# privacy-scaling-explorations/zkevm-specs

Measured on AMD Instinct MI355X. Metric: BN254 constraint-rows/sec, higher is better.
Workload: dtype u256 (BN254 Fr: 4xu64 canonical cells, u32-limb Montgomery); 1 GPU; EVM circuit, 2^18 execution steps per GPU, mixed-opcode synthetic trace (BASELINE configs[2]); RW table 816377 rows, bytecode table 43913 rows; steps_per_gpu=262144, rw_rows=816377, bytecode_rows=43913, witness_copies=3

## Files before the change

### zkevm_specs_amd/csrc/cpu_backend.cpp

```cpp
#include <stdio.h>
#include <string.h>
#include <chrono>
#include <functional>
#include <string>
#include <vector>

#include "../../include/zkevm_hip.h"
#include "dist_tally.hpp"
#include "state_circuit.hpp"
#include "evm_circuit.hpp"
#include "host_index.hpp"
#include "row_circuits.hpp"
#include "copy_circuit.hpp"
#include "sign_circuit.hpp"
#include "keccak_table.hpp"
#include "secp256k1.hpp"
#include "pi_circuit.hpp"
#include "state_assign.hpp"
#include "bytecode_assign.hpp"
#include "bytecode_code.hpp"
#include "block_tables.hpp"
#include "trace_witness.hpp"
#include "state_rekey.hpp"
#include "ecc_circuit.hpp"
// ... 384 lines not shown
    cpu_table(s->tab[1], t->bytecode, nullptr, t->n_bytecode, BYTECODE_NCELLS, bc_key_hash);
    cpu_table(s->tab[2], t->tx, t->tx_flags, t->n_tx, TX_NCELLS, tx_key_hash);
    cpu_table(s->tab[3], t->block, t->block_flags, t->n_block, BLOCK_NCELLS, blk_key_hash);
    cpu_table(s->tab[4], t->copy, nullptr, t->n_copy, COPY_T_NCELLS, copy_key_hash);
    cpu_table(s->tab[5], t->keccak, nullptr, t->n_keccak, KECCAK_NCELLS, keccak_key_hash);
    cpu_table(s->tab[6], t->exp, nullptr, t->n_exp, EXP_T_NCELLS, expt_key_hash);
    cpu_table(s->tab[7], t->sig, nullptr, t->n_sig, SIG_T_NCELLS, sig_key_hash);
    cpu_table(s->tab[8], t->ecc, nullptr, t->n_ecc, ECC_T_NCELLS, ecc_key_hash);
    cpu_table(s->tab[9], t->withdrawals, nullptr, t->n_withdrawals, 4, nullptr);
    a.rw = s->tab[0].t; a.bytecode = s->tab[1].t; a.tx = s->tab[2].t; a.block = s->tab[3].t; a.copy = s->tab[4].t;
    a.keccak = s->tab[5].t; a.exp = s->tab[6].t; a.sig = s->tab[7].t; a.ecc = s->tab[8].t; a.withdrawals = s->tab[9].t;
    {
        const HostEvmAgg g = evm_aggregates_host(t->tx, t->tx_flags, t->n_tx, t->withdrawals, t->n_withdrawals);
        a.agg_max_txs = g.max_txs; a.agg_total_txs = g.total_txs; a.agg_invalid_txs = g.invalid_txs;
        a.agg_bad_invalid_rows = g.bad_invalid_rows; a.agg_total_wds = g.total_wds;
        a.agg_rw_dups = rw_duplicate_rows_host(t->rw, t->n_rw);
    }
    a.aux = nullptr;
    a.aux_kind = nullptr;
    a.aux_cells = t->aux_cells ? t->aux_cells : 2u;
    if (t->aux && t->aux_kind) {
        s->aux64.assign(t->aux, t->aux + t->n_steps * a.aux_cells * 4);
        s->a32[1].assign(t->aux_kind, t->aux_kind + t->n_steps);
        a.aux = s->aux64.data();
        a.aux_kind = s->a32[1].data();
    }
    a.perm = nullptr;
    a.prof = nullptr;
    a.n_pairs = (u32)(t->n_steps - 1);
    a.opts = (t->begin_with_first_step ? 1u : 0u) | (t->end_with_last_step ? 2u : 0u);
    a.rw_dense = 0;
    a.rw_base = 0;
    a.rw_keys = nullptr;
    a.codes.n = 0;
    a.codes.mask = 0;
    a.codes.packed = nullptr;
    a.codes.entries = nullptr;
    a.codes.slots = nullptr;
    if (!(opts & ZK_OPT_GENERIC_INDEX)) {
        s->rw_meta = rw_dense_meta_host(s->tab[0].t.n ? s->tab[0].cells.data() : nullptr, t->n_rw);
        a.rw_dense = s->rw_meta.dense;
        a.rw_base = s->rw_meta.base;
        if (s->rw_meta.dense) {
            s->a64[1].resize((size_t)t->n_rw * 4);
            for (u64 r = 0; r < t->n_rw; r++) {
                const RwKey k = rw_pack_row(a.rw, (u32)r);
                for (int j = 0; j < 4; j++) s->a64[1][4 * r + j] = k.w[j];
            }
            a.rw_keys = s->a64[1].data();
        }
        if (t->n_bytecode) {
            build_code_dir(s->tab[1].cells.data(), t->n_bytecode, s->dir);
            a.codes.entries = s->dir.entries.data();
            a.codes.slots = s->dir.slots.data();
            a.codes.mask = s->dir.mask;
            a.codes.n = (u32)s->dir.entries.size();
            a.codes.packed = s->dir.packed.data();
        }
    }
    s->row = [s](u64 i) {
        u32 c = evm_check_step<EVM_GROUP_ALL>(s->evm, i);
        if (c == ZK_NOT_MINE) c = evm_check_step<EVM_GROUP_WARM>(s->evm, i);
        if (c == ZK_NOT_MINE) c = evm_check_step<EVM_GROUP_COLD>(s->evm, i);
        return c;
    };
    *out = s;
    return 0;
}
extern "C" int zk_evm_verify(const zk_evm_tables* t, uint32_t opts, uint32_t* status_out, zk_result* result) {
    ARG_TRY(result, "zk_evm_verify: result is null");
    zk_session* s = nullptr;
    const int rc = zk_evm_open(t, opts, &s);
    return rc ? rc : one_shot(s, status_out, result);
}

extern "C" int zk_evm_verify_batch(const zk_evm_tables* const* t, uint64_t n, uint32_t opts, zk_result* results) {
    ARG_TRY((t && results) || n == 0, "zk_evm_verify_batch: bad arguments");
    for (uint64_t i = 0; i < n; i++) ARG_TRY(t[i], "zk_evm_verify_batch: null witness");
    for (uint64_t i = 0; i < n; i++) {
        const int rc = zk_evm_verify(t[i], opts, nullptr, &results[i]);
        if (rc) return rc;
    }
// ... 1946 lines not shown
```

### zkevm_specs_amd/csrc/evm_circuit.hpp

```cpp
#pragma once
#include "common.hpp"
#include "evm_tables.h"
#include "keccak.hpp"
#include "secp_constants.h"
#include "bigz.hpp"

enum { S_STATE = 0, S_RWC, S_CALL_ID, S_IS_ROOT, S_IS_CREATE, S_CH_LO, S_CH_HI, S_PC, S_SP, S_GAS, S_MWS, S_REV, S_LOG, STEP_NCELLS };
enum { R_RWC = 0, R_RW, R_TAG, R_ID, R_ADDR, R_FT, R_KEY_LO, R_KEY_HI, R_VAL_LO, R_VAL_HI, R_PREV_LO, R_PREV_HI, R_AUX_LO, R_AUX_HI, RW_NCELLS };
enum { B_HASH_LO = 0, B_HASH_HI, B_TAG, B_INDEX, B_IS_CODE, B_VALUE, BYTECODE_NCELLS };
enum { TX_NCELLS = 5, BLOCK_NCELLS = 4 };
enum { CT_IS_FIRST = 0, CT_SRC_ID_LO, CT_SRC_ID_HI, CT_SRC_TAG, CT_DST_ID_LO, CT_DST_ID_HI, CT_DST_TAG, CT_SRC_ADDR,
       CT_SRC_ADDR_END, CT_DST_ADDR, CT_LENGTH, CT_RLC_ACC, CT_RWC, CT_RWC_INC, COPY_T_NCELLS };
enum { XT_IS_STEP = 0, XT_ID, XT_IS_LAST, XT_BASE0, XT_BASE1, XT_BASE2, XT_BASE3, XT_EXP_LO, XT_EXP_HI, XT_RES_LO, XT_RES_HI,
       EXP_T_NCELLS };
enum { SIG_T_NCELLS = 9, ECC_T_NCELLS = 13 };
enum { AUX_PAIR = 3, AUX_ECRECOVER = 5, AUX_ECADD = 6, AUX_ECMUL = 7, AUX_ECPAIRING = 8 };
enum { CDT_Bytecode = 1, CDT_Memory, CDT_TxCalldata, CDT_TxLog, CDT_RlcAcc };

struct EvmDyn {
    u32 rw_sparse;
    u32 codes_n;
    u64 rw_base;
    u32 codes_mask;
    u32 agg_max_txs, agg_total_txs, agg_invalid_txs, agg_bad_invalid_rows, agg_total_wds;
    u32 dir_entries;
    u32 n_deferred;
    u32 agg_rw_dups;
};

struct EvmArgs {
    const EvmDyn* dyn;
    const u64* steps;
    const u32* step_recs;
    u64 n_steps;
    ZkTable rw, bytecode, tx, block;
    ZkTable copy, keccak, exp;
    ZkTable sig, ecc;
    ZkTable withdrawals;
    u32 agg_max_txs, agg_total_txs, agg_invalid_txs, agg_bad_invalid_rows, agg_total_wds;
    u32 agg_rw_dups;
    const u64* aux;
    const u32* aux_kind;
    u32 aux_cells;
    u32 rw_dense;
    u64 rw_base;
    const u64* rw_keys;
    ZkCodeDir codes;
    unsigned long long* prof;
    u32* defer_list;
    u32* defer_count;
    const u32* perm;
    u32 n_pairs;
    u32 opts;
    u32* defer_count_twin;
};

ZK_HD void evm_args_resolve(EvmArgs& a) {
#ifdef EVM_RESOLVE_OFF
    return;
#endif
    if (a.dyn) {
        const EvmDyn d = *a.dyn;
        a.rw_dense = (a.rw.n != 0u && d.rw_sparse == 0u) ? 1u : 0u;
        a.rw_base = d.rw_base;
        a.codes.n = d.codes_n;
        a.codes.mask = d.codes_mask;
        a.agg_max_txs = d.agg_max_txs; a.agg_total_txs = d.agg_total_txs; a.agg_invalid_txs = d.agg_invalid_txs;
        a.agg_bad_invalid_rows = d.agg_bad_invalid_rows; a.agg_total_wds = d.agg_total_wds;
        a.agg_rw_dups = d.agg_rw_dups;
    }
}

#ifndef EVM_HOT_BLOCK
#define EVM_HOT_BLOCK 128
#endif
#define EVM_STAGE_LANES EVM_HOT_BLOCK
#define EV_PROF_WAVE ((blockIdx.x * blockDim.x + threadIdx.x) >> 6)
#define EV_PROF_ON(a) ((a).prof && (threadIdx.x & 63) == 0 && EV_PROF_WAVE < 4096u)
#define EVM_STAGE_STRIDE (EVM_STAGE_LANES + 1)
#define EVM_STAGE_ENTRIES 40
#define EVM_STAGE_GAS 10
ZK_HD constexpr int evm_stage_entry(int s, int c) {
    return c == S_CH_LO || c == S_CH_HI ? 24 + s * 8 + (c - S_CH_LO) * 4
           : s * 12 + (c < S_CH_LO ? c : c == S_PC ? 5 : c == S_SP ? 6 : c == S_MWS ? 7 : c == S_REV ? 8 : c == S_LOG ? 9 : EVM_STAGE_GAS);
}
#define EVM_DIR_MAX_SLOTS 128
#define EVM_DIR_MAX_ENTRIES 32
// ... 291 lines not shown
    Q.q[c] = v;
    Q.mask |= 1u << c;
}
ZK_HD void rwq_set_word(RwQ& Q, int c, const Word& w) {
    rwq_set(Q, c, w.lo);
    rwq_set(Q, c + 1, w.hi);
}
struct RwKey {
    u64 w[4];
};
ZK_HD bool rw_key_fields_fit(const Fr& rw, const Fr& tag, const Fr& id, const Fr& addr, const Fr& ft) {
    return fr_le_u64(rw, 255) && fr_le_u64(tag, 255) && fr_le_u64(ft, 255) && fr_fits64(id) && (addr.v[5] | addr.v[6] | addr.v[7]) == 0u;
}
ZK_HD RwKey rw_pack_fields(const Fr& rw, const Fr& tag, const Fr& id, const Fr& addr, const Fr& ft) {
    RwKey k;
    k.w[0] = (1ull << 63) | (u64)(rw.v[0] & 0xffu) | ((u64)(tag.v[0] & 0xffu) << 8) | ((u64)(ft.v[0] & 0xffu) << 16) | ((u64)addr.v[4] << 24);
    k.w[1] = fr_lo64(id);
    k.w[2] = fr_lo64(addr);
    k.w[3] = fr_hi64of128(addr);
    return k;
}
ZK_HD RwKey rw_pack_row(const ZkTable& t, u32 r) {
    const Fr rw = zk_table_cell(t, r, R_RW), tag = zk_table_cell(t, r, R_TAG), id = zk_table_cell(t, r, R_ID);
    const Fr addr = zk_table_cell(t, r, R_ADDR), ft = zk_table_cell(t, r, R_FT);
    if (!rw_key_fields_fit(rw, tag, id, addr, ft)) {
        RwKey k;
        k.w[0] = k.w[1] = k.w[2] = k.w[3] = 0;
        return k;
    }
    RwKey k = rw_pack_fields(rw, tag, id, addr, ft);
    k.w[0] |= (u64)((t.flags ? t.flags[r] : 3u) & 3u) << 56;
    return k;
}
ZK_HD u32 rw_dense_row(const EvmArgs& a, const Fr& rwc, bool& ok) {
    const u64 off = fr_lo64(rwc) - a.rw_base;
    ok = fr_fits64(rwc) && fr_lo64(rwc) >= a.rw_base && off < (u64)a.rw.n;
    return ok ? (u32)off : 0u;
}
struct RwRow {
    uint4 k01, k23;
    Fr v_lo, v_hi;
    u32 r;
};
template <int N>
struct RwRows {
    bool valid;
    RwRow row[N];
};
ZK_HD u32 rw_lookup(Ins& I, RwQ& Q, const Fr* rw_counter = nullptr, const RwRow* pre = nullptr) {
    if (rw_counter) {
        Q.q[R_RWC] = *rw_counter;
    } else {
        Q.q[R_RWC] = fr_add_u64(I.rwc, I.rw_off);
        I.rw_off++;
    }
    if (I.a->rw_dense) {
        I.seq++;
        bool ok;
        const u32 r = rw_dense_row(*I.a, Q.q[R_RWC], ok);
        bool key_cells = true;
#if EVM_FAST
        if (!I.a->rw_keys) I.defer = 3u;
#endif
        if (I.a->rw_keys) {
            uint4 k01, k23;
            if (pre) {
                if (pre->r != r && I.err == 0u) I.err = ZK_CODE(ZK_UNSUPPORTED, I.seq);
                k01 = pre->k01;
                k23 = pre->k23;
            } else {
                const uint4* kp = reinterpret_cast<const uint4*>(I.a->rw_keys + (u64)r * 4);
                k01 = kp[0];
                k23 = kp[1];
            }
            const u64 w0 = (u64)k01.x | ((u64)k01.y << 32), w1 = (u64)k01.z | ((u64)k01.w << 32);
            const u64 w2 = (u64)k23.x | ((u64)k23.y << 32), w3 = (u64)k23.z | ((u64)k23.w << 32);
            if (w0 >> 63) {
                const u32 m = Q.mask;
                if ((m >> R_RW) & 1u) ok = ok & (fr_le_u64(Q.q[R_RW], 255) & ((u32)(w0 & 0xffu) == Q.q[R_RW].v[0]));
                if ((m >> R_TAG) & 1u) ok = ok & (fr_le_u64(Q.q[R_TAG], 255) & ((u32)((w0 >> 8) & 0xffu) == Q.q[R_TAG].v[0]));
                if ((m >> R_FT) & 1u) ok = ok & (fr_le_u64(Q.q[R_FT], 255) & ((u32)((w0 >> 16) & 0xffu) == Q.q[R_FT].v[0]));
                if ((m >> R_ID) & 1u) ok = ok & (fr_fits64(Q.q[R_ID]) & (w1 == fr_lo64(Q.q[R_ID])));
                if ((m >> R_ADDR) & 1u) {
                    const Fr& qa = Q.q[R_ADDR];
                    ok = ok & (((qa.v[5] | qa.v[6] | qa.v[7]) == 0u) & (w2 == fr_lo64(qa)) & (w3 == fr_hi64of128(qa)) &
                               ((u32)((w0 >> 24) & 0xffffffffull) == qa.v[4]));
                }
                key_cells = false;
            }
        }
#if EVM_FAST
        if (key_cells) I.defer = 4u;
#else
        if (key_cells) {
#pragma unroll
            for (int c = 1; c <= R_FT; c++)
                if ((Q.mask >> c) & 1u) ok = ok & fr_eq(zk_table_cell(I.a->rw, r, c), Q.q[c]);
        }
#endif
#pragma unroll
        for (int c = R_FT + 1; c < RW_NCELLS; c++)
            if ((Q.mask >> c) & 1u) ok = ok & fr_eq(zk_table_cell(I.a->rw, r, c), Q.q[c]);
        if (!ok) ev_fail(I, ZK_LOOKUP_UNSAT);
        return r;
    }
    return table_lookup<RW_NCELLS>(I, I.a->rw, rw_key_hash_cell(Q.q[R_RWC]), Q.q, Q.mask);
}
template <int N>
ZK_HD void rw_rows_fetch_at(const Ins& I, RwRows<N>& R, u64 off) {
    const EvmArgs& a = *I.a;
    R.valid = a.rw_dense && a.rw_keys != nullptr;
    if (!R.valid) return;
#pragma unroll
    for (int k = 0; k < N; k++) {
        bool ok;
        const u32 r = rw_dense_row(a, fr_add_u64(I.rwc, off + (u64)k), ok);
        const uint4* kp = reinterpret_cast<const uint4*>(a.rw_keys + (u64)r * 4);
        R.row[k].k01 = kp[0];
        R.row[k].k23 = kp[1];
        R.row[k].r = r;
        R.row[k].v_lo = zk_table_cell(a.rw, r, R_VAL_LO);
        R.row[k].v_hi = zk_table_cell(a.rw, r, R_VAL_LO + 1);
    }
}
template <int N>
ZK_HD void rw_rows_fetch(const Ins& I, RwRows<N>& R) { rw_rows_fetch_at(I, R, I.rw_off); }
ZK_HD Fr rw_cell(const Ins& I, u32 row, int c) { return zk_table_cell(I.a->rw, row, c); }
ZK_HD Word rw_word(const Ins& I, u32 row, int c) { return word_of(rw_cell(I, row, c), rw_cell(I, row, c + 1)); }
ZK_HD WordOrValue rw_value(const Ins& I, u32 row) {
    WordOrValue v;
    v.w = rw_word(I, row, R_VAL_LO);
    v.is_word = I.a->rw.flags ? (I.a->rw.flags[row] & 1u) : true;
    return v;
}
ZK_HD WordOrValue rw_value_prev(const Ins& I, u32 row) {
    WordOrValue v;
    v.w = rw_word(I, row, R_PREV_LO);
    v.is_word = I.a->rw.flags ? (I.a->rw.flags[row] & 2u) : true;
    return v;
}

ZK_HD void code_dir_resolve(Ins& I, const Word& code_hash) {
    if (I.code_state != 0) return;
    const ZkCodeDir& dir = I.a->codes;
    I.code_state = 3;
#if !defined(ZK_HOSTSIM)
    static_assert(sizeof(ZkCodeEntry) == 96, "LDS mirror layout: 12 u64 per directory entry");
    if (dir.n != 0 && I.dir_lds && fr_fits128(code_hash.lo) && fr_fits128(code_hash.hi)) {
        u32 slot = (u32)zk_code_hash_key(code_hash.lo, code_hash.hi) & dir.mask;
        I.code_state = 2;
        const u64 h0 = fr_lo64(code_hash.lo), h1 = fr_hi64of128(code_hash.lo), h4 = fr_lo64(code_hash.hi), h5 = fr_hi64of128(code_hash.hi);
        for (u32 probes = 0; probes <= dir.mask; probes++) {
// ... 274 lines not shown
    RwQ Q;
    rwq_init(Q, rw, TG_Stack);
    rwq_set(Q, R_ID, I.call_id);
    const Fr& sp = I.sp;
    rwq_set(Q, R_ADDR, off >= 0 ? fr_add_u64(sp, (u64)off) : fr_sub_u64(sp, (u64)(-off)));
    rw_lookup(I, Q, nullptr, &row);
    return word_of(row.v_lo, row.v_hi);
}
template <int N>
ZK_HD Word stack_pop(Ins& I, const RwRows<N>& R, int k) {
    if (!R.valid) return stack_pop(I);
    int off = I.sp_off;
    I.sp_off++;
    return stack_lookup_row(I, 0, off, R.row[k]);
}
template <int N>
ZK_HD Word stack_push(Ins& I, const RwRows<N>& R, int k) {
    if (!R.valid) return stack_push(I);
    I.sp_off--;
    return stack_lookup_row(I, 1, I.sp_off, R.row[k]);
}
ZK_HD Fr memory_lookup(Ins& I, u32 rw, const Fr& addr, const Fr* call_id = nullptr) {
    RwQ Q;
    rwq_init(Q, rw, TG_Memory);
    rwq_set(Q, R_ID, call_id ? *call_id : I.call_id);
    rwq_set(Q, R_ADDR, addr);
    u32 r = rw_lookup(I, Q);
    return value_of(I, rw_value(I, r));
}
ZK_HD void memory_lookup_run32(Ins& I, u32 rw, const Fr& address) {
    const EvmArgs& a = *I.a;
    const Fr rwc0 = fr_add_u64(I.rwc, I.rw_off);
    const u64 off = fr_lo64(rwc0) - a.rw_base;
    bool fastpath = a.rw_dense && a.rw_keys && fr_fits64(rwc0) && fr_lo64(rwc0) >= a.rw_base && off + 32 <= (u64)a.rw.n && off + 32 > off &&
                    fr_fits64(I.call_id) && (address.v[5] | address.v[6] | address.v[7]) == 0u &&
                    !(address.v[4] == 0xffffffffu && address.v[3] == 0xffffffffu && address.v[2] == 0xffffffffu && address.v[1] == 0xffffffffu &&
                      address.v[0] >= 0xffffffe0u);
    u32 bad_lookup = 0, bad_type = 0;
    if (fastpath) {
        const uint4* kp = reinterpret_cast<const uint4*>(a.rw_keys + off * 4);
        const u64 id = fr_lo64(I.call_id);
#pragma unroll
        for (int b = 0; b < 4; b++) {
            uint4 k01[8], k23[8];
#pragma unroll
            for (int j = 0; j < 8; j++) { k01[j] = kp[2 * (8 * b + j)]; k23[j] = kp[2 * (8 * b + j) + 1]; }
#pragma unroll
            for (int j = 0; j < 8; j++) {
                const int k = 8 * b + j;
                const Fr ak = fr_add_u64(address, (u64)k);
                const u64 w0 = (u64)k01[j].x | ((u64)k01[j].y << 32), w1 = (u64)k01[j].z | ((u64)k01[j].w << 32);
                const u64 w2 = (u64)k23[j].x | ((u64)k23[j].y << 32), w3 = (u64)k23[j].z | ((u64)k23[j].w << 32);
                const u64 want0 = (1ull << 63) | (u64)rw | ((u64)TG_Memory << 8) | ((u64)ak.v[4] << 24);
                const u64 cmp_mask = ~((0xffull << 16) | (3ull << 56));
                if (!(w0 >> 63)) fastpath = false;
                const bool ok = ((w0 ^ want0) & cmp_mask) == 0 && w1 == id && w2 == fr_lo64(ak) && w3 == fr_hi64of128(ak);
                bad_lookup |= (ok ? 0u : 1u) << k;
                bad_type |= (u32)((w0 >> 56) & 1u) << k;
            }
        }
    }
    if (fastpath) {
        for (int k = 0; k < 32; k++) {
            I.seq++;
            if ((bad_lookup >> k) & 1u) ev_fail(I, ZK_LOOKUP_UNSAT);
            I.seq++;
            if ((bad_type >> k) & 1u) ev_fail(I, ZK_ASSERT);
        }
        I.rw_off += 32;
        return;
    }
    for (int k = 0; k < 32; k++) memory_lookup(I, rw, fr_add_u64(address, (u64)k));
}
ZK_HD WordOrValue call_context_lookup_word(Ins& I, u32 field_tag, u32 rw = 0, const Fr* call_id = nullptr) {
    RwQ Q;
    rwq_init(Q, rw, TG_CallContext);
    rwq_set(Q, R_ID, call_id ? *call_id : I.call_id);
    rwq_set(Q, R_ADDR, fr_u(field_tag));
    u32 r = rw_lookup(I, Q);
    return rw_value(I, r);
}
ZK_HD WordOrValue call_context_lookup_word_row(Ins& I, u32 field_tag, u32 rw, const Fr* call_id, const RwRow& row) {
    RwQ Q;
    rwq_init(Q, rw, TG_CallContext);
    rwq_set(Q, R_ID, call_id ? *call_id : I.call_id);
    rwq_set(Q, R_ADDR, fr_u(field_tag));
    const u32 r = rw_lookup(I, Q, nullptr, &row);
    WordOrValue v;
    v.w = word_of(row.v_lo, row.v_hi);
    const u64 w0 = (u64)row.k01.x | ((u64)row.k01.y << 32);
    v.is_word = (w0 >> 63) ? (((w0 >> 56) & 1ull) != 0ull) : (I.a->rw.flags ? (I.a->rw.flags[r] & 1u) : true);
    return v;
}
ZK_HD Fr call_context_lookup(Ins& I, u32 field_tag, u32 rw = 0, const Fr* call_id = nullptr) {
// ... 3580 lines not shown
```

### zkevm_specs_amd/csrc/zkevm_hip.hip

```cpp
#include <hip/hip_runtime.h>
#include <hip/hip_ext.h>
#include <stddef.h>
#include <stdio.h>
#include <string.h>
#include <stdlib.h>
#include <chrono>
#include <memory>
#include <string>
#include <vector>

#include <atomic>
#include <mutex>
#include <dlfcn.h>

#include "../../include/zkevm_hip.h"
#include "kernels.hpp"
#include "dist_tally.hpp"
#include "host_index.hpp"
#include "code_dir_build.hpp"

#define ZK_MAX_DEVICES 64
static std::mutex g_dev_mutex;
static hipStream_t g_own_stream[ZK_MAX_DEVICES] = {nullptr};
static hipStream_t g_batch_stream[ZK_MAX_DEVICES][2] = {{nullptr}};
// ... 220 lines not shown
        if (vblock == 0) {
            if ((k & 127u) == 0) group_start[k >> 7] = gsh[k >> 7] = excl;
            if (k == EVM_N_BINS - 1) group_start[EVM_N_GROUPS] = gsh[EVM_N_GROUPS] = src[k];
            for (u32 j = c_real; j < c; j++) perm[excl + j] = EVM_NO_PAIR;
        }
    }
    const u32 i = vblock * blockDim.x + threadIdx.x;
    u32 bin = 0, rank = 0;
    if (i < n_pairs) {
        bin = bin16[i];
        rank = atomicAdd(&local[bin], 1u);
    }
    __syncthreads();
    if (vblock == 0 && k == 0 && early_host) {
        __hip_atomic_store(&early_host[EVM_EARLY_WORD], gsh[EVM_GROUP_WARM + 1] - gsh[EVM_GROUP_WARM], __ATOMIC_RELAXED, __HIP_MEMORY_SCOPE_SYSTEM);
        __hip_atomic_store(&early_host[EVM_EARLY_WORD + 1], gsh[EVM_GROUP_COLD + 1] - gsh[EVM_GROUP_COLD], __ATOMIC_RELAXED, __HIP_MEMORY_SCOPE_SYSTEM);
        __threadfence_system();
        __hip_atomic_store(&early_host[EVM_EARLY_WORD + 2], early_seq, __ATOMIC_RELEASE, __HIP_MEMORY_SCOPE_SYSTEM);
    }
    if (k < EVM_N_BINS && local[k]) base[k] = excl + atomicAdd(&taken[k], local[k]);
    __syncthreads();
    if (i < n_pairs) perm[base[bin] + rank] = i;
}
__global__ __launch_bounds__(1024) void evm_state_scatter_kernel(const uint16_t* bin16, u32 n_pairs, const u32* hist, u32* hist_next,
                                                                 u32* taken, u32* group_start, u32* perm) {
    evm_state_scatter_body(blockIdx.x, bin16, n_pairs, hist, hist_next, taken, group_start, perm);
}
__global__ __launch_bounds__(256) void evm_open_fill_kernel(uint4* ff, u64 n_ff, uint4* zero, u64 n_zero) {
    const u64 stride = (u64)gridDim.x * blockDim.x;
    const uint4 F = make_uint4(~0u, ~0u, ~0u, ~0u), Z = make_uint4(0u, 0u, 0u, 0u);
    for (u64 i = (u64)blockIdx.x * blockDim.x + threadIdx.x; i < n_ff; i += stride) ff[i] = F;
    for (u64 i = (u64)blockIdx.x * blockDim.x + threadIdx.x; i < n_zero; i += stride) zero[i] = Z;
}
__device__ __forceinline__ void rw_prepare_quad(const ZkTable& t, u64* keys, EvmDyn* dyn, u32 vthread, u32 sparse_bit = 1u) {
    const u32 r = vthread >> 2, q = vthread & 3u;
    const bool in = r < t.n;
    uint4 c0 = make_uint4(0, 0, 0, 0), c1 = c0, c2 = c0;
    u64 base = 0;
    u32 flags = 3u;
    if (in) {
        const uint4* p = reinterpret_cast<const uint4*>(t.cells + (u64)r * RW_NCELLS * 4) + q;
        c0 = p[0];
        c1 = p[4];
        c2 = p[8];
        if (q == 0) {
            base = t.cells[0];
            if (t.flags) flags = t.flags[r];
        }
    }
    bool fit, dense_ok;
    u64 w0 = 0, w1 = 0, w2 = 0, w3 = 0;
    const bool z0hi = (c0.y | c0.z | c0.w) == 0u, z1hi = (c1.y | c1.z | c1.w) == 0u, z2hi = (c2.y | c2.z | c2.w) == 0u;
    const bool z0 = z0hi && c0.x == 0u, z1 = z1hi && c1.x == 0u, z2 = z2hi && c2.x == 0u;
    if (q == 0) {
        const u64 rwc = (u64)c0.x | ((u64)c0.y << 32);
        dense_ok = (c0.z | c0.w) == 0u && rwc == base + r && base + r >= base;
        fit = z1hi && c1.x <= 255u;
        w0 = (u64)(c1.x & 0xffu) << 8 | ((u64)(flags & 3u) << 56) | (1ull << 63);
        w2 = (u64)c2.x | ((u64)c2.y << 32);
        w3 = (u64)c2.z | ((u64)c2.w << 32);
    } else if (q == 1) {
        dense_ok = z0;
        fit = z1 && z2hi;
        w0 = (u64)c2.x << 24;
    } else if (q == 2) {
        dense_ok = true;
        fit = z0hi && c0.x <= 255u && (c1.z | c1.w) == 0u && z2hi && c2.x <= 255u;
        w0 = (u64)(c0.x & 0xffu) | ((u64)(c2.x & 0xffu) << 16);
        w1 = (u64)c1.x | ((u64)c1.y << 32);
    } else {
        dense_ok = true;
        fit = z0 && z1 && z2;
    }
    const u32 qshift = threadIdx.x & 60u;
    const bool fits = ((__ballot(fit) >> qshift) & 0xfull) == 0xfull;
    const unsigned long long nd = __ballot(in && !dense_ok);
    if (nd != 0ull && (threadIdx.x & 63u) == 0) atomicOr(&dyn->rw_sparse, sparse_bit);
    if (r == 0 && q == 0 && in) dyn->rw_base = base;
#pragma unroll
    for (int m = 1; m <= 2; m <<= 1) {
        w0 |= __shfl_xor(w0, m);
        w1 |= __shfl_xor(w1, m);
        w2 |= __shfl_xor(w2, m);
        w3 |= __shfl_xor(w3, m);
    }
    if (!fits) w0 = w1 = w2 = w3 = 0;
    if (in && q < 2) {
        const u64 a = q == 0 ? w0 : w2, b2 = q == 0 ? w1 : w3;
        reinterpret_cast<uint4*>(keys + (u64)r * 4)[q] = make_uint4((u32)a, (u32)(a >> 32), (u32)b2, (u32)(b2 >> 32));
    }
}
#define EVM_OPEN_TABLES 8
struct EvmOpenTables {
    ZkTable t[EVM_OPEN_TABLES];
    u32 block_start[EVM_OPEN_TABLES + 2];
    const u64* wds;
    u32 n_wds;
    EvmDyn* dyn;
    ZkTally* tally;
    ZkTable rw;
    u64* rw_keys;
    u32 dir_block0, rw_block0;
    DirBuild dir;
    const u64* steps;
    u32 n_steps;
    u32* step_recs;
    u32 rec_block0;
    EvmSortArgs sort;
    u32 hist_block0;
    u32 lat_period;
    u32 tail_row0, tail_blocks;
#ifdef ZK_DIAG_P1
    u32 diag_skip;
#endif
};
__device__ __forceinline__ void evm_open_small_tables(const EvmOpenTables& o, u32 block) {
    int k = 0;
#pragma unroll
    for (int j = 1; j <= EVM_OPEN_TABLES; j++) k += block >= o.block_start[j] ? 1 : 0;
    const u32 r = (block - o.block_start[k]) * blockDim.x + threadIdx.x;
    if (k == EVM_OPEN_TABLES) {
        const bool nz = r < o.n_wds && !fr_is_zero(fr_load(o.wds + ((u64)r * 4 + 3) * 4));
        const unsigned long long b = __ballot(nz);
        if (b && (threadIdx.x & 63u) == 0) atomicAdd(&o.dyn->agg_total_wds, (u32)__popcll(b));
        return;
    }
    const ZkTable& t = o.t[k];
    const bool in = r < t.n;
    if (k == 0) {
        bool caller = false, present = false, invalid = false, bad = false;
        if (in) {
            const Fr tag = zk_table_cell(t, r, 1), lo = zk_table_cell(t, r, 3), hi = zk_table_cell(t, r, 4);
            caller = fr_eq_u64(tag, 4);
            present = caller && !(fr_is_zero(lo) && fr_is_zero(hi));
// ... 14 lines not shown
    switch (k) {
    case 0: h = tx_key_hash(t, r); break;
    case 1: h = blk_key_hash(t, r); break;
    case 2: h = bc_key_hash(t, r); break;
    case 3: h = copy_key_hash(t, r); break;
    case 4: h = keccak_key_hash(t, r); break;
    case 5: h = expt_key_hash(t, r); break;
    case 6: h = sig_key_hash(t, r); break;
    default: h = ecc_key_hash(t, r); break;
    }
    u32* slots = const_cast<u32*>(t.slots);
    u32 s = (u32)h & t.mask;
    while (atomicCAS(&slots[s], ZK_EMPTY_SLOT, r) != ZK_EMPTY_SLOT) s = (s + 1) & t.mask;
}
__global__ __launch_bounds__(256) void evm_open_phase1_kernel(EvmOpenTables o) {
    if (blockIdx.x == 0 && threadIdx.x < 2) {
        o.tally[threadIdx.x].fail_count = 0ull;
        o.tally[threadIdx.x].first_fail = ~0ull;
    }
    u32 b = blockIdx.x;
    if (o.lat_period > 1u && b < o.rec_block0) {
        const u32 q = b / o.lat_period;
        b = (b == q * o.lat_period && q < o.rw_block0) ? q : o.rw_block0 + b - (q + 1u < o.rw_block0 ? q + 1u : o.rw_block0);
    }
#ifdef ZK_DIAG_P1
    {
        const u32 range = b < o.dir_block0 ? 1u : b < o.hist_block0 ? 2u : b < o.rw_block0 ? 4u : b < o.rec_block0 ? 8u : 16u;
        if (o.diag_skip & range) return;
    }
#endif
    if (b < o.dir_block0) evm_open_small_tables(o, b);
    else if (b < o.hist_block0) dirb_events_row(o.dir, (b - o.dir_block0) * blockDim.x + threadIdx.x);
    else if (b < o.rw_block0) evm_state_hist_body(b - o.hist_block0, o.sort.steps, o.sort.n_pairs, o.sort.hist, o.sort.taken, o.sort.bin16, o.sort.tally, o.sort.defer_count);
    else if (b < o.rec_block0) rw_prepare_quad(o.rw, o.rw_keys, o.dyn, (b - o.rw_block0) * blockDim.x + threadIdx.x);
    else evm_step_record_quad(o.steps, o.n_steps, o.step_recs, (b - o.rec_block0) * blockDim.x + threadIdx.x);
}
#define EVM_OPEN_RW_GENERIC_BLOCKS 64u
#define EVM_OPEN_P2_BLOCK 1024u
__global__ __launch_bounds__(1024) void evm_open_phase2_kernel(EvmOpenTables o, u32 scatter_blocks, u32 dir_blocks, u32 force_generic) {
    if (blockIdx.x < scatter_blocks) {
        evm_state_scatter_body(blockIdx.x, o.sort.bin16, o.sort.n_pairs, o.sort.hist, o.sort.hist_next, o.sort.taken, o.sort.group_start, o.sort.perm,
                               o.sort.early_host, o.sort.early_seq);
        return;
    }
    const u32 b = blockIdx.x - scatter_blocks;
    if (b < dir_blocks) {
        dirb_finalize_entry(o.dir, b * blockDim.x + threadIdx.x);
        return;
    }
    const u32 generic_blocks = gridDim.x - scatter_blocks - dir_blocks - o.tail_blocks;
    if (b >= dir_blocks + generic_blocks) {
        rw_prepare_quad(o.rw, o.rw_keys, o.dyn, o.tail_row0 * 4u + (b - dir_blocks - generic_blocks) * blockDim.x + threadIdx.x, 2u);
        return;
    }
    if (!force_generic && (o.dyn->rw_sparse & 1u) == 0u) return;
    if (force_generic && b == dir_blocks && threadIdx.x == 0) o.dyn->rw_sparse = 1u;
    u32* slots = const_cast<u32*>(o.rw.slots);
    const u32 stride = generic_blocks * blockDim.x;
    for (u32 r = (b - dir_blocks) * blockDim.x + threadIdx.x; r < o.rw.n; r += stride) {
        u32 s = (u32)rw_key_hash(o.rw, r) & o.rw.mask;
        bool dup = false;
        for (;;) {
            const u32 q = atomicCAS(&slots[s], ZK_EMPTY_SLOT, r);
            if (q == ZK_EMPTY_SLOT) break;
            if (!dup && q < o.rw.n) {
                bool same = true;
                for (int c = 0; c < RW_NCELLS && same; c++) same = fr_eq(zk_table_cell(o.rw, q, c), zk_table_cell(o.rw, r, c));
                dup = same;
            }
            s = (s + 1) & o.rw.mask;
        }
        if (dup) atomicAdd(&o.dyn->agg_rw_dups, 1u);
    }
}

__global__ void fr_op_kernel(int op, const u64* a, const u64* b, u64* out, u64 n) {
    u64 i = (u64)blockIdx.x * blockDim.x + threadIdx.x;
    if (i >= n) return;
    Fr x = fr_load(a + 4 * i), y = fr_load(b + 4 * i), r;
    switch (op) {
    case 0: r = fr_add(x, y); break;
    case 1: r = fr_sub(x, y); break;
    case 2: r = fr_mul(x, y); break;
    case 3: r = fr_mont(x, y); break;
    case 4: r = fr_neg(x); break;
// ... 531 lines not shown
        const size_t zero_bytes = dyn_bytes + 2 * hist_bytes + status_bytes + 3 * (size_t)cap_big * 4;
        char* zero = nullptr;
        if ((rc = dev_alloc(s, (void**)&zero, zero_bytes))) goto fail;
        EvmResultBlock* const rb = (EvmResultBlock*)zero;
        EvmDyn* dyn = &rb->dyn;
        s->d_result = rb;
        if ((rc = arena_pinned(s->device, &s->h_result))) goto fail;
        {
            void* hd = nullptr;
            if (hipHostGetDevicePointer(&hd, s->h_result, 0) == hipSuccess) s->h_result_dev = (u32*)hd;
            (void)hipGetLastError();
        }
        static_assert(sizeof(EvmResultBlock) <= 256, "the result block outgrew its slot");
        static_assert((EVM_N_BINS * sizeof(u32)) % 16 == 0, "zero region pieces are 16-byte multiples");
        s->d_hist = (u32*)(zero + dyn_bytes);
        s->d_hist2 = (u32*)(zero + dyn_bytes + hist_bytes);
        s->d_status = no_status ? nullptr : (u32*)(zero + dyn_bytes + 2 * hist_bytes);
        u32* const dir_last = (u32*)(zero + dyn_bytes + 2 * hist_bytes + status_bytes);
        E.dyn = dyn;
        E.defer_count = &dyn->n_deferred;
        if ((rc = dev_alloc(s, (void**)&E.defer_list, (size_t)E.n_pairs * sizeof(u32)))) goto fail;
        s->d_tally = rb->tally;
        s->tally_last = s->d_tally;
        {
            const u64 n16 = n_ff / 4 + zero_bytes / 16;
            const u32 fill_grid = (u32)(n16 / 256 < 2048 ? (n16 + 255) / 256 : 2048);
            if (arena_event(s->device, &s->ev_open0) || arena_event(s->device, &s->ev_open1)) s->ev_open0 = s->ev_open1 = nullptr;
            hipExtLaunchKernelGGL(evm_open_fill_kernel, dim3(fill_grid ? fill_grid : 1u), dim3(256), 0, s->stream, s->ev_open0, nullptr, 0, (uint4*)ff,
                                  (u64)(n_ff / 4), (uint4*)zero, (u64)(zero_bytes / 16));
        }
        E.rw_dense = 0;
        E.rw_base = 0;
        E.rw_keys = nullptr;
        E.codes.n = 0;
        E.codes.mask = 0;
        E.codes.packed = nullptr;
        E.codes.entries = nullptr;
        E.codes.slots = nullptr;
        E.agg_max_txs = E.agg_total_txs = E.agg_invalid_txs = E.agg_bad_invalid_rows = E.agg_total_wds = E.agg_rw_dups = 0;
        EvmOpenTables o;
        memset(&o, 0, sizeof o);
        u32 blk = 0;
        for (int k = 0; k < EVM_OPEN_TABLES; k++) { o.t[k] = *small[k]; o.block_start[k] = blk; blk += (small[k]->n + 255u) / 256u; }
        o.block_start[EVM_OPEN_TABLES] = blk;
        blk += (u32)((t->n_withdrawals + 255) / 256);
        o.block_start[EVM_OPEN_TABLES + 1] = blk;
        o.wds = E.withdrawals.cells;
        o.n_wds = (u32)t->n_withdrawals;
        o.dyn = dyn;
        o.tally = s->d_tally;
        o.rw = E.rw;
        if (t->n_rw && !generic) {
            u64* d_keys = nullptr;
            if ((rc = dev_alloc(s, (void**)&d_keys, (size_t)t->n_rw * 32))) goto fail;
            E.rw_keys = d_keys;
            o.rw_keys = d_keys;
        }
        u64 n_head = t->n_rw;
        if ((internal & EVM_OPEN_ONESHOT) && o.rw_keys && t->n_rw < (1ull << 30)) {
            static const u32 tail_pm = [] { const char* e = getenv("ZK_P2_RW_TAIL"); const int v = e ? atoi(e) : ZK_P2_RW_TAIL_DEFAULT; return (u32)(v < 0 ? 0 : v > 999 ? 999 : v); }();
            const u64 h = (t->n_rw - t->n_rw * tail_pm / 1000 + 63) & ~63ull;
            if (h < t->n_rw) n_head = h;
        }
        const u32 rw_row_blocks = o.rw_keys ? (u32)((n_head + 63) / 64) : 0u;
        if (n_head < t->n_rw) {
            o.tail_row0 = (u32)n_head;
            o.tail_blocks = (u32)((t->n_rw - n_head + EVM_OPEN_P2_BLOCK / 4 - 1) / (EVM_OPEN_P2_BLOCK / 4));
        }
        o.dir_block0 = blk;
        u32 dir_row_blocks = 0;
        if (want_dir) {
            DirBuild& d = o.dir;
            d.rows = E.bytecode.cells;
            d.n = (u32)t->n_bytecode;
            d.rep = dir_rep;
            d.first = dir_first;
            d.last = dir_last;
            d.runs = dir_last + cap_big;
            d.bad = dir_last + 2 * (size_t)cap_big;
            d.big_mask = cap_big - 1;
            d.small_slots = small_slots;
            d.dyn = dyn;
            if ((rc = dev_alloc(s, (void**)&d.packed, (size_t)d.n * sizeof(uint16_t)))) goto fail;
            if ((rc = dev_alloc(s, (void**)&d.entries, (size_t)DIRB_MAX_ENTRIES * sizeof(ZkCodeEntry)))) goto fail;
            if ((rc = dev_alloc(s, (void**)&d.list, (size_t)DIRB_MAX_ENTRIES * 4))) goto fail;
            dir_row_blocks = (d.n + 255u) / 256u;
            E.codes.entries = d.entries;
            E.codes.slots = d.small_slots;
// ... 3436 lines not shown
```

Measured before the change: 1.656 billion rows/s.

## Split RW lookup keys into a 16-byte primary and an optional high half

```diff
diff --git a/zkevm_specs_amd/csrc/cpu_backend.cpp b/zkevm_specs_amd/csrc/cpu_backend.cpp
--- a/zkevm_specs_amd/csrc/cpu_backend.cpp
+++ b/zkevm_specs_amd/csrc/cpu_backend.cpp
@@ -440,6 +440,7 @@
     a.rw_dense = 0;
     a.rw_base = 0;
     a.rw_keys = nullptr;
+    a.rw_keys16 = a.rw_keys_hi = nullptr;
     a.codes.n = 0;
     a.codes.mask = 0;
     a.codes.packed = nullptr;
@@ -451,11 +452,24 @@
         a.rw_base = s->rw_meta.base;
         if (s->rw_meta.dense) {
             s->a64[1].resize((size_t)t->n_rw * 4);
+#if ZK_RW_KEY16
+            u64* const lo = s->a64[1].data();
+            u64* const hi = lo + (size_t)t->n_rw * 2;
+            for (u64 r = 0; r < t->n_rw; r++) {
+                const RwKey16 k = rw_pack_row16(a.rw, (u32)r);
+                lo[2 * r] = k.a0;
+                lo[2 * r + 1] = k.a1;
+                if (rw_key16_wide(k.a0)) { hi[2 * r] = k.h0; hi[2 * r + 1] = k.h1; }
+            }
+            a.rw_keys16 = lo;
+            a.rw_keys_hi = hi;
+#else
             for (u64 r = 0; r < t->n_rw; r++) {
                 const RwKey k = rw_pack_row(a.rw, (u32)r);
                 for (int j = 0; j < 4; j++) s->a64[1][4 * r + j] = k.w[j];
             }
             a.rw_keys = s->a64[1].data();
+#endif
         }
         if (t->n_bytecode) {
             build_code_dir(s->tab[1].cells.data(), t->n_bytecode, s->dir);
diff --git a/zkevm_specs_amd/csrc/evm_circuit.hpp b/zkevm_specs_amd/csrc/evm_circuit.hpp
--- a/zkevm_specs_amd/csrc/evm_circuit.hpp
+++ b/zkevm_specs_amd/csrc/evm_circuit.hpp
@@ -53,6 +53,8 @@
     u32 n_pairs;
     u32 opts;
     u32* defer_count_twin;
+    const u64* rw_keys16;
+    const u64* rw_keys_hi;
 };
 
 ZK_HD void evm_args_resolve(EvmArgs& a) {
@@ -410,13 +412,88 @@
     k.w[0] |= (u64)((t.flags ? t.flags[r] : 3u) & 3u) << 56;
     return k;
 }
+#ifndef ZK_RW_KEY16
+#define ZK_RW_KEY16 1
+#endif
+#if !ZK_RW_KEY16 || defined(ZK_HOSTSIM)
+#define RW_KEY32_COMPILED 1
+#else
+#define RW_KEY32_COMPILED 0
+#endif
+#ifndef RW_KEY16_HI_SELECT
+#if EVM_FAST
+#define RW_KEY16_HI_SELECT 0
+#else
+#define RW_KEY16_HI_SELECT 1
+#endif
+#endif
+struct RwKey16 {
+    u64 a0, a1, h0, h1;
+};
+ZK_HD bool rw_key16_fits(u64 a0) { return (a0 >> 63) != 0ull; }
+ZK_HD bool rw_key16_wide(u64 a0) { return (a0 >> 62) == 2ull; }
+ZK_HD RwKey16 rw_key16_finish(bool fits, u64 a0, u64 a1, u64 h0, u64 h1) {
+    RwKey16 k;
+    if (!fits) {
+        k.a0 = k.a1 = k.h0 = k.h1 = 0;
+        return k;
+    }
+    k.a0 = a0 | (1ull << 63) | ((h0 | h1) == 0ull ? 1ull << 62 : 0ull);
+    k.a1 = a1;
+    k.h0 = h0;
+    k.h1 = h1;
+    return k;
+}
+ZK_HD RwKey16 rw_pack_row16(const ZkTable& t, u32 r) {
+    const Fr rw = zk_table_cell(t, r, R_RW), tag = zk_table_cell(t, r, R_TAG), id = zk_table_cell(t, r, R_ID);
+    const Fr addr = zk_table_cell(t, r, R_ADDR), ft = zk_table_cell(t, r, R_FT);
+    const u64 a0 = (u64)(rw.v[0] & 0xffu) | ((u64)(tag.v[0] & 0xffu) << 8) | ((u64)(ft.v[0] & 0xffu) << 16) | ((u64)id.v[0] << 24) |
+                   ((u64)((t.flags ? t.flags[r] : 3u) & 3u) << 56);
+    return rw_key16_finish(rw_key_fields_fit(rw, tag, id, addr, ft), a0, fr_lo64(addr), (u64)id.v[1] | ((u64)addr.v[4] << 32), fr_hi64of128(addr));
+}
+ZK_HD bool rw_query_wants_high(const Fr* q, u32 mask) {
+    const bool id_narrow = ((mask >> R_ID) & 1u) && fr_fits64(q[R_ID]) && q[R_ID].v[1] == 0u;
+    const Fr& qa = q[R_ADDR];
+    const bool addr_narrow = ((mask >> R_ADDR) & 1u) && fr_fits64(qa);
+    return !(id_narrow && addr_narrow);
+}
+ZK_HD bool rw_key16_match(u64 a0, u64 a1, u64 h0, u64 h1, const Fr* q, u32 m) {
+    const bool wide = rw_key16_wide(a0);
+    if (!wide) h0 = h1 = 0ull;
+    bool ok = !(wide && !rw_query_wants_high(q, m));
+    if ((m >> R_RW) & 1u) ok = ok & (fr_le_u64(q[R_RW], 255) & ((u32)(a0 & 0xffu) == q[R_RW].v[0]));
+    if ((m >> R_TAG) & 1u) ok = ok & (fr_le_u64(q[R_TAG], 255) & ((u32)((a0 >> 8) & 0xffu) == q[R_TAG].v[0]));
+    if ((m >> R_FT) & 1u) ok = ok & (fr_le_u64(q[R_FT], 255) & ((u32)((a0 >> 16) & 0xffu) == q[R_FT].v[0]));
+    if ((m >> R_ID) & 1u) ok = ok & (fr_fits64(q[R_ID]) & ((u32)(a0 >> 24) == q[R_ID].v[0]) & ((u32)h0 == q[R_ID].v[1]));
+    if ((m >> R_ADDR) & 1u) {
+        const Fr& qa = q[R_ADDR];
+        ok = ok & (((qa.v[5] | qa.v[6] | qa.v[7]) == 0u) & (a1 == fr_lo64(qa)) & (h1 == fr_hi64of128(qa)) & ((u32)(h0 >> 32) == qa.v[4]));
+    }
+    return ok;
+}
+ZK_HD bool rw_keys16_on(const EvmArgs& a) {
+#if ZK_RW_KEY16
+    return a.rw_keys16 != nullptr;
+#else
+    return false;
+#endif
+}
+ZK_HD bool rw_keys_any(const EvmArgs& a) {
+#if RW_KEY32_COMPILED
+    if (a.rw_keys) return true;
+#endif
+    return rw_keys16_on(a);
+}
 ZK_HD u32 rw_dense_row(const EvmArgs& a, const Fr& rwc, bool& ok) {
     const u64 off = fr_lo64(rwc) - a.rw_base;
     ok = fr_fits64(rwc) && fr_lo64(rwc) >= a.rw_base && off < (u64)a.rw.n;
     return ok ? (u32)off : 0u;
 }
 struct RwRow {
-    uint4 k01, k23;
+    uint4 k01;
+#if RW_KEY32_COMPILED
+    uint4 k23;
+#endif
     Fr v_lo, v_hi;
     u32 r;
 };
@@ -438,9 +515,33 @@
         const u32 r = rw_dense_row(*I.a, Q.q[R_RWC], ok);
         bool key_cells = true;
 #if EVM_FAST
-        if (!I.a->rw_keys) I.defer = 3u;
-#endif
-        if (I.a->rw_keys) {
+        if (!rw_keys_any(*I.a)) I.defer = 3u;
+#endif
+#if ZK_RW_KEY16
+        if (I.a->rw_keys16) {
+            const bool want_hi = rw_query_wants_high(Q.q, Q.mask);
+            uint4 k, h;
+            h.x = h.y = h.z = h.w = 0u;
+            if (pre) {
+                if (pre->r != r && I.err == 0u) I.err = ZK_CODE(ZK_UNSUPPORTED, I.seq);
+                k = pre->k01;
+            } else {
+                k = reinterpret_cast<const uint4*>(I.a->rw_keys16)[r];
+            }
+#if RW_KEY16_HI_SELECT
+            h = reinterpret_cast<const uint4*>(want_hi ? I.a->rw_keys_hi : I.a->rw_keys16)[r];
+#else
+            if (want_hi) h = reinterpret_cast<const uint4*>(I.a->rw_keys_hi)[r];
+#endif
+            const u64 a0 = (u64)k.x | ((u64)k.y << 32), a1 = (u64)k.z | ((u64)k.w << 32);
+            if (rw_key16_fits(a0)) {
+                ok = ok & rw_key16_match(a0, a1, (u64)h.x | ((u64)h.y << 32), (u64)h.z | ((u64)h.w << 32), Q.q, Q.mask);
+                key_cells = false;
+            }
+        }
+#endif
+#if RW_KEY32_COMPILED
+        if (!rw_keys16_on(*I.a) && I.a->rw_keys) {
             uint4 k01, k23;
             if (pre) {
                 if (pre->r != r && I.err == 0u) I.err = ZK_CODE(ZK_UNSUPPORTED, I.seq);
@@ -467,6 +568,7 @@
                 key_cells = false;
             }
         }
+#endif
 #if EVM_FAST
         if (key_cells) I.defer = 4u;
 #else
@@ -487,15 +589,25 @@
 template <int N>
 ZK_HD void rw_rows_fetch_at(const Ins& I, RwRows<N>& R, u64 off) {
     const EvmArgs& a = *I.a;
-    R.valid = a.rw_dense && a.rw_keys != nullptr;
+    R.valid = a.rw_dense && rw_keys_any(a);
     if (!R.valid) return;
+    const bool k16 = rw_keys16_on(a);
 #pragma unroll
     for (int k = 0; k < N; k++) {
         bool ok;
         const u32 r = rw_dense_row(a, fr_add_u64(I.rwc, off + (u64)k), ok);
-        const uint4* kp = reinterpret_cast<const uint4*>(a.rw_keys + (u64)r * 4);
-        R.row[k].k01 = kp[0];
-        R.row[k].k23 = kp[1];
+#if RW_KEY32_COMPILED
+        if (!k16) {
+            const uint4* kp = reinterpret_cast<const uint4*>(a.rw_keys + (u64)r * 4);
+            R.row[k].k01 = kp[0];
+            R.row[k].k23 = kp[1];
+        } else {
+            R.row[k].k23.x = R.row[k].k23.y = R.row[k].k23.z = R.row[k].k23.w = 0u;
+        }
+#endif
+#if ZK_RW_KEY16
+        if (k16) R.row[k].k01 = reinterpret_cast<const uint4*>(a.rw_keys16)[r];
+#endif
         R.row[k].r = r;
         R.row[k].v_lo = zk_table_cell(a.rw, r, R_VAL_LO);
         R.row[k].v_hi = zk_table_cell(a.rw, r, R_VAL_LO + 1);
@@ -836,12 +948,39 @@
     const EvmArgs& a = *I.a;
     const Fr rwc0 = fr_add_u64(I.rwc, I.rw_off);
     const u64 off = fr_lo64(rwc0) - a.rw_base;
-    bool fastpath = a.rw_dense && a.rw_keys && fr_fits64(rwc0) && fr_lo64(rwc0) >= a.rw_base && off + 32 <= (u64)a.rw.n && off + 32 > off &&
+    bool fastpath = a.rw_dense && rw_keys_any(a) && fr_fits64(rwc0) && fr_lo64(rwc0) >= a.rw_base && off + 32 <= (u64)a.rw.n && off + 32 > off &&
                     fr_fits64(I.call_id) && (address.v[5] | address.v[6] | address.v[7]) == 0u &&
                     !(address.v[4] == 0xffffffffu && address.v[3] == 0xffffffffu && address.v[2] == 0xffffffffu && address.v[1] == 0xffffffffu &&
                       address.v[0] >= 0xffffffe0u);
     u32 bad_lookup = 0, bad_type = 0;
-    if (fastpath) {
+#if ZK_RW_KEY16
+    if (rw_keys16_on(a)) {
+        fastpath = fastpath && I.call_id.v[1] == 0u && fr_fits64(address) && fr_lo64(address) <= ~31ull;
+        if (fastpath) {
+            const uint4* kp = reinterpret_cast<const uint4*>(a.rw_keys16) + off;
+            const u64 want0 = (3ull << 62) | (u64)rw | ((u64)TG_Memory << 8) | ((u64)I.call_id.v[0] << 24);
+            const u64 cmp_mask = ~((0xffull << 16) | (3ull << 56));
+            const u64 addr0 = fr_lo64(address);
+#pragma unroll
+            for (int b = 0; b < 4; b++) {
+                uint4 kk[8];
+#pragma unroll
+                for (int j = 0; j < 8; j++) kk[j] = kp[8 * b + j];
+#pragma unroll
+                for (int j = 0; j < 8; j++) {
+                    const int k = 8 * b + j;
+                    const u64 a0 = (u64)kk[j].x | ((u64)kk[j].y << 32), a1 = (u64)kk[j].z | ((u64)kk[j].w << 32);
+                    if ((a0 >> 62) != 3ull) fastpath = false;
+                    const bool ok = ((a0 ^ want0) & cmp_mask) == 0 && a1 == addr0 + (u64)k;
+                    bad_lookup |= (ok ? 0u : 1u) << k;
+                    bad_type |= (u32)((a0 >> 56) & 1u) << k;
+                }
+            }
+        }
+    }
+#endif
+#if RW_KEY32_COMPILED
+    if (fastpath && !rw_keys16_on(a)) {
         const uint4* kp = reinterpret_cast<const uint4*>(a.rw_keys + off * 4);
         const u64 id = fr_lo64(I.call_id);
 #pragma unroll
@@ -864,6 +1003,7 @@
             }
         }
     }
+#endif
     if (fastpath) {
         for (int k = 0; k < 32; k++) {
             I.seq++;
diff --git a/zkevm_specs_amd/csrc/zkevm_hip.hip b/zkevm_specs_amd/csrc/zkevm_hip.hip
--- a/zkevm_specs_amd/csrc/zkevm_hip.hip
+++ b/zkevm_specs_amd/csrc/zkevm_hip.hip
@@ -276,7 +276,7 @@
     for (u64 i = (u64)blockIdx.x * blockDim.x + threadIdx.x; i < n_ff; i += stride) ff[i] = F;
     for (u64 i = (u64)blockIdx.x * blockDim.x + threadIdx.x; i < n_zero; i += stride) zero[i] = Z;
 }
-__device__ __forceinline__ void rw_prepare_quad(const ZkTable& t, u64* keys, EvmDyn* dyn, u32 vthread, u32 sparse_bit = 1u) {
+__device__ __forceinline__ void rw_prepare_quad(const ZkTable& t, u64* keys, u64* keys_hi, EvmDyn* dyn, u32 vthread, u32 sparse_bit = 1u) {
     const u32 r = vthread >> 2, q = vthread & 3u;
     const bool in = r < t.n;
     uint4 c0 = make_uint4(0, 0, 0, 0), c1 = c0, c2 = c0;
@@ -300,18 +300,33 @@
         const u64 rwc = (u64)c0.x | ((u64)c0.y << 32);
         dense_ok = (c0.z | c0.w) == 0u && rwc == base + r && base + r >= base;
         fit = z1hi && c1.x <= 255u;
+#if ZK_RW_KEY16
+        w0 = (u64)(c1.x & 0xffu) << 8 | ((u64)(flags & 3u) << 56);
+        w1 = (u64)c2.x | ((u64)c2.y << 32);
+        w3 = (u64)c2.z | ((u64)c2.w << 32);
+#else
         w0 = (u64)(c1.x & 0xffu) << 8 | ((u64)(flags & 3u) << 56) | (1ull << 63);
         w2 = (u64)c2.x | ((u64)c2.y << 32);
         w3 = (u64)c2.z | ((u64)c2.w << 32);
+#endif
     } else if (q == 1) {
         dense_ok = z0;
         fit = z1 && z2hi;
+#if ZK_RW_KEY16
+        w2 = (u64)c2.x << 32;
+#else
         w0 = (u64)c2.x << 24;
+#endif
     } else if (q == 2) {
         dense_ok = true;
         fit = z0hi && c0.x <= 255u && (c1.z | c1.w) == 0u && z2hi && c2.x <= 255u;
         w0 = (u64)(c0.x & 0xffu) | ((u64)(c2.x & 0xffu) << 16);
+#if ZK_RW_KEY16
+        w0 |= (u64)c1.x << 24;
+        w2 = (u64)c1.y;
+#else
         w1 = (u64)c1.x | ((u64)c1.y << 32);
+#endif
     } else {
         dense_ok = true;
         fit = z0 && z1 && z2;
@@ -328,11 +343,17 @@
         w2 |= __shfl_xor(w2, m);
         w3 |= __shfl_xor(w3, m);
     }
+#if ZK_RW_KEY16
+    const RwKey16 k = rw_key16_finish(fits, w0, w1, w2, w3);
+    if (in && q == 0) reinterpret_cast<uint4*>(keys)[r] = make_uint4((u32)k.a0, (u32)(k.a0 >> 32), (u32)k.a1, (u32)(k.a1 >> 32));
+    if (in && q == 1 && rw_key16_wide(k.a0)) reinterpret_cast<uint4*>(keys_hi)[r] = make_uint4((u32)k.h0, (u32)(k.h0 >> 32), (u32)k.h1, (u32)(k.h1 >> 32));
+#else
     if (!fits) w0 = w1 = w2 = w3 = 0;
     if (in && q < 2) {
         const u64 a = q == 0 ? w0 : w2, b2 = q == 0 ? w1 : w3;
         reinterpret_cast<uint4*>(keys + (u64)r * 4)[q] = make_uint4((u32)a, (u32)(a >> 32), (u32)b2, (u32)(b2 >> 32));
     }
+#endif
 }
 #define EVM_OPEN_TABLES 8
 struct EvmOpenTables {
@@ -344,6 +365,7 @@
     ZkTally* tally;
     ZkTable rw;
     u64* rw_keys;
+    u64* rw_keys_hi;
     u32 dir_block0, rw_block0;
     DirBuild dir;
     const u64* steps;
@@ -424,7 +446,7 @@
     if (b < o.dir_block0) evm_open_small_tables(o, b);
     else if (b < o.hist_block0) dirb_events_row(o.dir, (b - o.dir_block0) * blockDim.x + threadIdx.x);
     else if (b < o.rw_block0) evm_state_hist_body(b - o.hist_block0, o.sort.steps, o.sort.n_pairs, o.sort.hist, o.sort.taken, o.sort.bin16, o.sort.tally, o.sort.defer_count);
-    else if (b < o.rec_block0) rw_prepare_quad(o.rw, o.rw_keys, o.dyn, (b - o.rw_block0) * blockDim.x + threadIdx.x);
+    else if (b < o.rec_block0) rw_prepare_quad(o.rw, o.rw_keys, o.rw_keys_hi, o.dyn, (b - o.rw_block0) * blockDim.x + threadIdx.x);
     else evm_step_record_quad(o.steps, o.n_steps, o.step_recs, (b - o.rec_block0) * blockDim.x + threadIdx.x);
 }
 #define EVM_OPEN_RW_GENERIC_BLOCKS 64u
@@ -442,7 +464,7 @@
     }
     const u32 generic_blocks = gridDim.x - scatter_blocks - dir_blocks - o.tail_blocks;
     if (b >= dir_blocks + generic_blocks) {
-        rw_prepare_quad(o.rw, o.rw_keys, o.dyn, o.tail_row0 * 4u + (b - dir_blocks - generic_blocks) * blockDim.x + threadIdx.x, 2u);
+        rw_prepare_quad(o.rw, o.rw_keys, o.rw_keys_hi, o.dyn, o.tail_row0 * 4u + (b - dir_blocks - generic_blocks) * blockDim.x + threadIdx.x, 2u);
         return;
     }
     if (!force_generic && (o.dyn->rw_sparse & 1u) == 0u) return;
@@ -1040,6 +1062,7 @@
         E.rw_dense = 0;
         E.rw_base = 0;
         E.rw_keys = nullptr;
+        E.rw_keys16 = E.rw_keys_hi = nullptr;
         E.codes.n = 0;
         E.codes.mask = 0;
         E.codes.packed = nullptr;
@@ -1061,7 +1084,13 @@
         if (t->n_rw && !generic) {
             u64* d_keys = nullptr;
             if ((rc = dev_alloc(s, (void**)&d_keys, (size_t)t->n_rw * 32))) goto fail;
+#if ZK_RW_KEY16
+            E.rw_keys16 = d_keys;
+            E.rw_keys_hi = d_keys + (size_t)t->n_rw * 2;
+            o.rw_keys_hi = d_keys + (size_t)t->n_rw * 2;
+#else
             E.rw_keys = d_keys;
+#endif
             o.rw_keys = d_keys;
         }
         u64 n_head = t->n_rw;
```

Result: slower. 1.533 billion rows/s (-7.4%).
